# uberalex974/Reinforcement-Learning

Measured on AMD Instinct MI355X. Metric: env-steps/sec (whole node) at 32768 arenas; PPO wall-clock per 1M steps, higher is better.
Workload: dtype f32

## Files before the change

### include/rlgpu_ppo.h

```cpp
#ifndef RLGPU_PPO_H
#define RLGPU_PPO_H

#include <stdint.h>
#include "rlgpu_core.h"

#ifdef __cplusplus
extern "C" {
#endif

#define RLGPU_MAX_LAYERS 8

typedef struct {
    int32_t obs_size;
    int32_t num_actions;
    int32_t policy_layers[RLGPU_MAX_LAYERS];
    int32_t n_policy_layers;
    int32_t critic_layers[RLGPU_MAX_LAYERS];
    int32_t n_critic_layers;
    int32_t layer_norm;
    float leaky_slope;
    int32_t activation;
    float policy_lr, critic_lr;
    float beta1, beta2, eps, weight_decay;
    float clip_range;
// ... 8 lines not shown
    int64_t sample_row_offset;
    float policy_temperature;
    int32_t mask_entropy;
} rlgpu_ppo_config;

enum { RLGPU_GEMM_F32X6 = 0, RLGPU_GEMM_F32 = 1, RLGPU_GEMM_F16X3 = 2 };
enum { RLGPU_ACT_LEAKY_RELU = 0, RLGPU_ACT_RELU = 1, RLGPU_ACT_SIGMOID = 2, RLGPU_ACT_TANH = 3 };
enum { RLGPU_INFER_BF16 = 0, RLGPU_INFER_F16 = 1, RLGPU_INFER_F32 = 2 };

typedef struct rlgpu_ppo rlgpu_ppo;

enum {
    RLGPU_M_ENTROPY = 0, RLGPU_M_KL, RLGPU_M_POLICY_LOSS, RLGPU_M_CRITIC_LOSS, RLGPU_M_RATIO,
    RLGPU_M_CLIP_FRACTION, RLGPU_M_COUNT, RLGPU_M_GRAD_NORM_POLICY, RLGPU_M_GRAD_NORM_CRITIC,
    RLGPU_M_GRAD_NORM_SHARED, RLGPU_M_GUIDING_LOSS = 10 ,
    RLGPU_M_TL_LOSS = 11, RLGPU_M_TL_ACCURACY = 12, RLGPU_M_TL_OLD_ENTROPY = 13,
    RLGPU_M_TL_UPDATE_MAGNITUDE = 14,
    RLGPU_NUM_METRICS = 16
};

int rlgpu_ppo_create(const rlgpu_ppo_config* cfg, rlgpu_ppo** out);
int rlgpu_ppo_destroy(rlgpu_ppo* h);
int32_t rlgpu_ppo_config_size(void);
int rlgpu_ppo_get_config(rlgpu_ppo* h, rlgpu_ppo_config* out);

int rlgpu_ppo_buffers(rlgpu_ppo* h, float** d_params, float** d_grads, int64_t* num_params);
int rlgpu_ppo_model_range(rlgpu_ppo* h, int32_t model, int64_t* offset, int64_t* count);
int rlgpu_ppo_init_params(rlgpu_ppo* h, uint64_t seed, void* stream);
int rlgpu_ppo_refresh_half(rlgpu_ppo* h, void* stream);

int rlgpu_debug_infer_trace(void* d_buf, int64_t capacity);
int rlgpu_kernel_timing(int32_t enable);
int rlgpu_kernel_timing_read(double* ms, double* work, int64_t* count, int32_t nslots);

int rlgpu_ppo_forward(rlgpu_ppo* h, int32_t model, int32_t precision, const float* d_in, int32_t n,
                      float* d_out, void* stream);

int rlgpu_ppo_infer_actions(rlgpu_ppo* h, const float* d_obs, const uint8_t* d_masks, int32_t n,
                            int32_t deterministic, uint64_t rng_step, int32_t* d_actions, float* d_logp,
                            void* stream);
int rlgpu_ppo_set_version(rlgpu_ppo* h, const float* d_policy_params, void* stream);
int rlgpu_ppo_infer_actions_mixed(rlgpu_ppo* h, const float* d_obs, const uint8_t* d_masks, int32_t n,
                                  int32_t deterministic, uint64_t rng_step, const uint8_t* d_old_rows,
                                  int32_t* d_actions, float* d_logp, void* stream);
int rlgpu_ppo_set_guide(rlgpu_ppo* h, const float* d_policy_params, void* stream);
int rlgpu_ppo_infer_guide_logits(rlgpu_ppo* h, const float* d_obs, int64_t n, uint16_t* d_logits16, void* stream);
int rlgpu_ppo_infer_actions_rows(rlgpu_ppo* h, const float* d_obs, const uint8_t* d_masks, int32_t n, int64_t row0,
                                 int32_t deterministic, uint64_t rng_step, const uint8_t* d_old_rows,
                                 int32_t* d_actions, float* d_logp, void* stream);
int rlgpu_ppo_fused_infer(rlgpu_ppo* h, int32_t model);
int rlgpu_ppo_wave_infer(rlgpu_ppo* h, int32_t model);
int rlgpu_ppo_infer_actions_wave(rlgpu_ppo* h, const float* d_obs, const uint8_t* d_masks, int32_t n, int64_t row0,
                                 int32_t deterministic, uint64_t rng_step, const uint8_t* d_old_rows,
                                 int32_t* d_actions, float* d_logp, void* stream);
int rlgpu_ppo_infer_values_wave(rlgpu_ppo* h, int32_t model, const float* d_obs, int32_t n, float* d_out, void* stream);
int rlgpu_ppo_infer_critic(rlgpu_ppo* h, const float* d_obs, int64_t n, float* d_values, void* stream);

int rlgpu_mean_std(const float* d_x, int64_t n, float* d_out, void* stream);

int rlgpu_ppo_minibatch(rlgpu_ppo* h, const float* d_obs, const uint8_t* d_masks, const int32_t* d_actions,
                        const float* d_old_logp, const float* d_adv, const float* d_target,
                        const int32_t* d_index, int64_t start, int32_t n, int64_t batch_size,
                        const float* d_adv_stats, float* d_metrics, void* stream);

int rlgpu_ppo_minibatch_guided(rlgpu_ppo* h, const float* d_obs, const uint8_t* d_masks, const int32_t* d_actions,
                               const float* d_old_logp, const float* d_adv, const float* d_target,
// ... 42 lines not shown
```

### reinforcement-learning_amd/csrc/mlp_kernels.hpp

```cpp
#pragma once
#include <hip/hip_bf16.h>
#include <hip/hip_fp16.h>
#include <hip/hip_runtime.h>
#include <stdint.h>

#include <cstdlib>

namespace mlp {

#define DEV __device__ __forceinline__

typedef float f32x16 __attribute__((ext_vector_type(16)));
typedef short bf16x8 __attribute__((ext_vector_type(8)));

enum { A_IK = 0, A_KI = 1 };
enum { B_JK = 0, B_KJ = 1 };

constexpr int BM = 128, BN = 128, BK = 32;
constexpr int KP = 4;
constexpr int MP = 4;

struct GemmArgs {
    const float* A;
    const float* B;
// ... 1147 lines not shown
                for (int q = 0; q < MAXH; q++) {
                    const int c = lcol<MAXH>(lane, q);
                    v[r][q] = c < H ? z[c] : 0.f;
                }
            }
        }
        lnf_rows<MAXH, RF, ACT>(v, row, R, H, g, b, slope, use_ln, vec, lane, act, stats, vmax, head_w, head_b, head_out);
    }
    if (amax) h3_amax_commit(amax, vmax);
}

constexpr int RLN_BM = 64, RLN_J = 512, RLN_ZP = RLN_J + 8;
constexpr int RLN_LDS = 32 * RLN_ZP * 4;
static_assert(2 * 2 * RLN_BM * 32 * 2 <= RLN_LDS, "the A stages must fit the z stage");
__global__ void __launch_bounds__(256) frag_weight_h3(const uint16_t* planes, int64_t plane, int ld, uint16_t* frag) {
    const int e = blockIdx.x * 256 + threadIdx.x;
    if (e >= (ld / 16) * (RLN_J / 32) * 2 * 64) return;
    const int lane = e & 63, p = (e >> 6) & 1, jb = (e >> 7) % (RLN_J / 32), ks = (e >> 7) / (RLN_J / 32);
    const uint16_t* src = planes + p * plane + (int64_t)(jb * 32 + (lane & 31)) * ld + ks * 16 + 8 * (lane >> 5);
    *reinterpret_cast<u32x4_t*>(frag + (int64_t)e * 8) = *reinterpret_cast<const u32x4_t*>(src);
}
struct RowLnArgs {
    const float* gamma;
    const float* beta;
    float slope;
    int use_ln;
    float* act;
    float2* stats;
    float* amax;
    const float* head_w;
    const float* head_b;
    float* head_out;
};
DEV int h3_row_kloop(const GemmArgs& g, unsigned char* smem, f32x16 (&acc)[2][4]) {
    constexpr int KSTEP = (RLN_J / 32) * 2 * 64 * 8;
    auto As = reinterpret_cast<uint16_t (*)[2][RLN_BM][XK]>(smem);
    const int t = threadIdx.x, lane = t & 63, w = t >> 6;
    const int i0 = blockIdx.x * RLN_BM;
    const int ke = g.K;
#pragma unroll
    for (int a = 0; a < 2; a++)
#pragma unroll
        for (int b = 0; b < 4; b++)
#pragma unroll
            for (int r = 0; r < 16; r++) acc[a][b][r] = 0.f;
    const int srow = t / XKG, kg = t % XKG;
    const float* arow = i0 + srow < g.I ? g.A + (int64_t)(i0 + srow) * g.lda : nullptr;
    f32x4_t va[2];
    const int pa = h3_pow(shard_max_bits(g.amax_a));
    const float sa = pow2f(pa);
    auto load_a = [&](int k0) {
        va[0] = load4v<true>(arow, k0 + kg * 8, ke);
        va[1] = load4v<true>(arow, k0 + kg * 8 + 4, ke);
    };
    auto store_a = [&](int buf) {
        u32x4_t h, l;
        split2h(va, sa, h, l);
        const int c = xchunk<XK>(srow, kg) * 8;
        *reinterpret_cast<u32x4_t*>(&As[buf][0][srow][c]) = h;
        *reinterpret_cast<u32x4_t*>(&As[buf][1][srow][c]) = l;
    };
    const uint16_t* Bw = reinterpret_cast<const uint16_t*>(g.B) + (w * 4 * 2 * 64 + lane) * 8;
    const int last = (int)g.ldb / 16 - 1;
    auto load_b = [&](h16x8 (&b)[2][4], int s) {
        const uint16_t* q = Bw + (int64_t)min(s, last) * KSTEP;
#pragma unroll
        for (int tj = 0; tj < 4; tj++)
#pragma unroll
            for (int p = 0; p < 2; p++) b[p][tj] = *reinterpret_cast<const h16x8*>(q + (tj * 2 + p) * 64 * 8);
    };
    const int l32 = lane & 31, hh = lane >> 5;
    auto mfma_step = [&](int buf, int ks, const h16x8 (&b)[2][4]) {
        const int kc = 2 * ks + hh;
        h16x8 a[2][2];
#pragma unroll
        for (int p = 0; p < 2; p++)
#pragma unroll
            for (int u = 0; u < 2; u++) a[p][u] = kc_frag(As[buf][p], l32 + 32 * u, kc);
        h3_mfma_step<4>(a, b, acc);
    };
    h16x8 b0[2][4], b1[2][4];
    load_a(0);
    load_b(b0, 0);
    store_a(0);
    __syncthreads();
    load_a(XK);
    int buf = 0;
    for (int k0 = 0; k0 < ke; k0 += XK) {
        const int s = k0 / 16;
        load_b(b1, s + 1);
        __builtin_amdgcn_sched_barrier(0);
        mfma_step(buf, 0, b0);
        __builtin_amdgcn_sched_barrier(0);
        load_b(b0, s + 2);
        __builtin_amdgcn_sched_barrier(0);
        mfma_step(buf, 1, b1);
        store_a(buf ^ 1);
        load_a(k0 + 2 * XK);
        __syncthreads();
        buf ^= 1;
    }
    return pa;
}
__global__ void __launch_bounds__(256, 2) gemm_h3_rowln(GemmArgs g, RowLnArgs ln) {
    constexpr int MAXH = RLN_J / 64, RF = lnf_rf<MAXH>();
    __shared__ __attribute__((aligned(16))) unsigned char smem[RLN_LDS];
    float* zs = reinterpret_cast<float*>(smem);
    const int t = threadIdx.x, lane = t & 63, w = t >> 6;
    const int i0 = blockIdx.x * RLN_BM;
    const int l32 = lane & 31, hh = lane >> 5;
    f32x16 acc[2][4];
    const int pa = h3_row_kloop(g, smem, acc);
    float csc[4], bj[4];
#pragma unroll
    for (int tj = 0; tj < 4; tj++) {
        const int j = w * 128 + tj * 32 + l32;
        csc[tj] = g.bscale[j];
        bj[tj] = g.bias ? g.bias[j] : 0.f;
    }
    float lg[MAXH], lb[MAXH];
    lnf_affine<MAXH>(ln.gamma, ln.beta, RLN_J, ln.use_ln, lane, lg, lb);
    uint32_t vmax = 0;
#pragma unroll
    for (int ti = 0; ti < 2; ti++) {
        if (ti) __syncthreads();
#pragma unroll
        for (int tj = 0; tj < 4; tj++)
#pragma unroll
            for (int r = 0; r < 16; r++) {
                const float v = acc[ti][tj][r] + 0.f;
                zs[((r & 3) + 8 * (r >> 2) + 4 * hh) * RLN_ZP + w * 128 + tj * 32 + l32] = h3_out(v, csc[tj], pa, bj[tj]);
            }
        __syncthreads();
        for (int b0 = 0; b0 < 32 / 4; b0 += RF) {
            int row[RF];
            float v[RF][MAXH];
#pragma unroll
            for (int r = 0; r < RF; r++) {
                const int zr = w * (32 / 4) + b0 + r;
                row[r] = i0 + ti * 32 + zr;
#pragma unroll
                for (int q = 0; q < MAXH; q += 4) {
                    const int c = lcol<MAXH>(lane, q);
                    const float4 x = *reinterpret_cast<const float4*>(zs + zr * RLN_ZP + c);
                    v[r][q] = x.x; v[r][q + 1] = x.y; v[r][q + 2] = x.z; v[r][q + 3] = x.w;
                    if (row[r] < g.I) *reinterpret_cast<float4*>(g.C + (int64_t)row[r] * g.ldc + c) = x;
                }
            }
            lnf_rows<MAXH, RF>(v, row, g.I, RLN_J, lg, lb, ln.slope, ln.use_ln, true, lane, ln.act, ln.stats, vmax, ln.head_w,
                               ln.head_b, ln.head_out);
        }
    }
    if (ln.amax) h3_amax_commit(ln.amax, vmax);
}

template <int MAXH>
DEV int hcol(int lane, int q) {
    return MAXH >= 8 ? 8 * lane + 512 * (q >> 3) + (q & 7) : MAXH * lane + q;
}
template <int MAXH, bool F16, int ACT = ACT_LEAKY>
__global__ void __launch_bounds__(256) ln_act_fwd_bf16(const uint16_t* Z, const uint16_t* gamma, const uint16_t* beta, int R,
                                                      int H, float slope, int use_ln, uint16_t* out) {
    const int wv = threadIdx.x >> 6, lane = threadIdx.x & 63;
    const bool vec = (H % 8 == 0) && (MAXH % 8 == 0);
    float g[MAXH], b[MAXH];
#pragma unroll
    for (int q = 0; q < MAXH; q++) {
        const int c = hcol<MAXH>(lane, q);
        g[q] = (use_ln && c < H) ? h2f<F16>(gamma[c]) : 1.f;
        b[q] = (use_ln && c < H) ? h2f<F16>(beta[c]) : 0.f;
    }
    for (int i = 0; i < LNF_ROWS / 4; i++) {
        const int row = blockIdx.x * LNF_ROWS + i * 4 + wv;
        if (row >= R) break;
        const uint16_t* z = Z + (int64_t)row * H;
        float v[MAXH];
        if (vec) {
#pragma unroll
            for (int q = 0; q < MAXH; q += 8) {
                const int c = hcol<MAXH>(lane, q);
                u32x4 t = {0u, 0u, 0u, 0u};
                if (c < H) t = *reinterpret_cast<const u32x4*>(z + c);
#pragma unroll
                for (int k = 0; k < 4; k++) {
                    v[q + 2 * k] = h2f<F16>((uint16_t)(t[k] & 0xffffu));
                    v[q + 2 * k + 1] = h2f<F16>((uint16_t)(t[k] >> 16));
                }
// ... 178 lines not shown
        red[w][2][c] = pb[q];
    }
    __syncthreads();
    if (HEAD) {
#pragma unroll
        for (int q = 0; q < MAXH; q++) hred[w][lcol<MAXH>(lane, q)] = ph[q];
        if (lane == 0) hred[w][64 * MAXH] = phb;
    }
    __syncthreads();
    float* out = part + (int64_t)blockIdx.x * 3 * H;
    for (int k = 0; k < 3; k++)
        for (int c = threadIdx.x; c < H; c += 256)
            out[k * H + c] = red[0][k][c] + red[1][k][c] + red[2][k][c] + red[3][k][c];
    if (HEAD) {
        float* ho = head_part + (int64_t)blockIdx.x * (H + 1);
        for (int c = threadIdx.x; c < H; c += 256) ho[c] = hred[0][c] + hred[1][c] + hred[2][c] + hred[3][c];
        if (threadIdx.x == 0)
            ho[H] = hred[0][64 * MAXH] + hred[1][64 * MAXH] + hred[2][64 * MAXH] + hred[3][64 * MAXH];
    }
    if (amax) h3_amax_commit(amax, vmax);
}

struct RowLnBwdArgs {
    const float* gamma;
    const float* beta;
    float slope;
    int use_ln;
    const float* z;
    const float2* stats;
    float* dz;
    float* part;
    float* amax;
};
__global__ void __launch_bounds__(256, 2) gemm_h3_row_lnbwd(GemmArgs g, RowLnBwdArgs ln) {
    constexpr int MAXH = RLN_J / 64, PR = 2;
    const int H = g.J;
    static_assert(4 * 3 * RLN_J * 4 <= RLN_LDS, "the wave partials must fit the dA stage");
    __shared__ __attribute__((aligned(16))) unsigned char smem[RLN_LDS];
    float* zs = reinterpret_cast<float*>(smem);
    auto red = reinterpret_cast<float (*)[3][RLN_J]>(smem);
    const int t = threadIdx.x, lane = t & 63, w = t >> 6;
    const int i0 = blockIdx.x * RLN_BM;
    const int l32 = lane & 31, hh = lane >> 5;
    f32x16 acc[2][4];
    const int pa = h3_row_kloop(g, smem, acc);
    float csc[4];
#pragma unroll
    for (int tj = 0; tj < 4; tj++) csc[tj] = g.bscale[w * 128 + tj * 32 + l32];
    uint32_t vmax = 0;
#pragma unroll
    for (int ti = 0; ti < 2; ti++) {
        const int r0 = i0 + ti * 32;
        if (ti) {
            if (r0 >= g.I) break;
            __syncthreads();
        }
#pragma unroll
        for (int tj = 0; tj < 4; tj++)
#pragma unroll
            for (int r = 0; r < 16; r++) {
                const float v = acc[ti][tj][r] + 0.f;
                zs[((r & 3) + 8 * (r >> 2) + 4 * hh) * RLN_ZP + w * 128 + tj * 32 + l32] = h3_out(v, csc[tj], pa, 0.f);
            }
        __syncthreads();
        float lg[MAXH], lb[MAXH], pg[MAXH], pb[MAXH], pz[MAXH], ph[MAXH];
        float phb = 0.f;
        lnf_affine<MAXH>(ln.gamma, ln.beta, H, ln.use_ln, lane, lg, lb);
#pragma unroll
        for (int q = 0; q < MAXH; q++) pg[q] = pb[q] = pz[q] = ph[q] = 0.f;
        for (int rr = w; rr < 32; rr += 4 * PR) {
            float xs[PR][MAXH], as[PR][MAXH];
            float2 sts[PR];
#pragma unroll
            for (int j = 0; j < PR; j++) {
                const int row = r0 + rr + 4 * j;
                const int rw = row < g.I ? row : g.I - 1;
                const float* xh = ln.z + (int64_t)rw * H;
                sts[j] = ln.stats[rw];
#pragma unroll
                for (int q = 0; q < MAXH; q += 4) {
                    const int c = lcol<MAXH>(lane, q);
                    const float4 x = *reinterpret_cast<const float4*>(xh + c);
                    const float4 u = *reinterpret_cast<const float4*>(zs + (rr + 4 * j) * RLN_ZP + c);
                    xs[j][q] = x.x; xs[j][q + 1] = x.y; xs[j][q + 2] = x.z; xs[j][q + 3] = x.w;
                    as[j][q] = u.x; as[j][q + 1] = u.y; as[j][q + 2] = u.z; as[j][q + 3] = u.w;
                }
            }
#pragma unroll
            for (int j = 0; j < PR; j++) {
                const int row = r0 + rr + 4 * j;
                if (row >= g.I) break;
                lnb_row<MAXH, false>(xs[j], as[j], sts[j], 0.f, lg, lb, ln.slope, ln.use_ln, H, true, lane,
                                     ln.dz + (int64_t)row * H, pz, pg, pb, ph, phb, vmax);
            }
        }
        __syncthreads();
#pragma unroll
        for (int q = 0; q < MAXH; q += 4) {
            const int c = lcol<MAXH>(lane, q);
            *reinterpret_cast<float4*>(&red[w][0][c]) = make_float4(pz[q], pz[q + 1], pz[q + 2], pz[q + 3]);
            *reinterpret_cast<float4*>(&red[w][1][c]) = make_float4(pg[q], pg[q + 1], pg[q + 2], pg[q + 3]);
            *reinterpret_cast<float4*>(&red[w][2][c]) = make_float4(pb[q], pb[q + 1], pb[q + 2], pb[q + 3]);
        }
        __syncthreads();
        float* out = ln.part + (int64_t)(2 * blockIdx.x + ti) * 3 * H;
#pragma unroll
        for (int k = 0; k < 3; k++)
#pragma unroll
            for (int c = t; c < H; c += 256) out[k * H + c] = red[0][k][c] + red[1][k][c] + red[2][k][c] + red[3][k][c];
    }
    if (ln.amax) h3_amax_commit(ln.amax, vmax);
}

constexpr int LNW_ROWS = 32;
DEV int wcol(int k) { return 4 * (int)threadIdx.x + 1024 * k; }
DEV float4 ld4(const float* p, int c, int H) { return c < H ? *reinterpret_cast<const float4*>(p + c) : make_float4(0.f, 0.f, 0.f, 0.f); }

template <int NV, int ACT = ACT_LEAKY, int LNW_RB = 4>
__global__ void __launch_bounds__(256) ln_act_fwd_wide(const float* Z, const float* gamma, const float* beta, int R, int H,
                                                      float slope, int use_ln, float* act, float2* stats, float* amax,
                                                      const float*, const float*, float*) {
    __shared__ float red[2][LNW_RB][4];
    const int w = threadIdx.x >> 6;
    uint32_t vmax = 0;
    float4 g[NV], b[NV];
#pragma unroll
    for (int k = 0; k < NV; k++) {
        g[k] = use_ln ? ld4(gamma, wcol(k), H) : make_float4(1.f, 1.f, 1.f, 1.f);
        b[k] = use_ln ? ld4(beta, wcol(k), H) : make_float4(0.f, 0.f, 0.f, 0.f);
    }
    const int r_end = min(R, (int)(blockIdx.x + 1) * LNW_ROWS);
    for (int r0 = blockIdx.x * LNW_ROWS; r0 < r_end; r0 += LNW_RB) {
        float4 v[LNW_RB][NV];
#pragma unroll
        for (int j = 0; j < LNW_RB; j++) {
            const float* z = Z + (int64_t)min(r0 + j, R - 1) * H;
#pragma unroll
            for (int k = 0; k < NV; k++) v[j][k] = ld4(z, wcol(k), H);
        }
        float mean[LNW_RB], rs[LNW_RB];
#pragma unroll
        for (int j = 0; j < LNW_RB; j++) {
            mean[j] = 0.f;
            rs[j] = 1.f;
        }
// ... 312 lines not shown
```

### reinforcement-learning_amd/csrc/ppo.hip

```cpp
#include <hipcub/hipcub.hpp>

#include <cmath>
#include <cstring>
#include <type_traits>
#include <vector>

#include "../../include/rlgpu_ppo.h"
#include "common.hpp"
#include "mlp_kernels.hpp"
#include "ppo_kernels.hpp"
#include "infer_kernels.hpp"

namespace {

using rlgpu::ceil_div;

#define RLGPU_H16_LAUNCH(F16, KERN, ...)                                                     \
    do {                                                                                     \
        if (F16) hipLaunchKernelGGL(KERN<true>, __VA_ARGS__);                                \
        else hipLaunchKernelGGL(KERN<false>, __VA_ARGS__);                                   \
    } while (0)

struct Side {
    int64_t planes = -1;
// ... 81 lines not shown
    int nm = 2;
    bool shared() const { return nm == 3; }
    float* dshared = nullptr;
    int64_t nparams = 0, nhalf = 0;
    float *params = nullptr, *grads = nullptr, *exp_avg = nullptr, *exp_avg_sq = nullptr;
    uint16_t* half = nullptr;
    uint16_t* half_ver = nullptr;
    uint16_t *frag = nullptr, *frag_ver = nullptr;
    int64_t nfrag = 0;
    bool has_ver = false;
    uint16_t *half_guide = nullptr, *frag_guide = nullptr;
    float* guide_f = nullptr;
    bool has_guide = false;
    float* teach_f = nullptr;
    bool split_dirty[3] = {true, true, true};
    int64_t step[3] = {0, 0, 0};
    int32_t opt[3] = {RLGPU_OPT_ADAMW, RLGPU_OPT_ADAMW, RLGPU_OPT_ADAMW};
    bool opt_stepped[3] = {false, false, false};
    int hmax = 0;
    float *scratch = nullptr;
    hipStream_t aux = nullptr;
    hipEvent_t ev_fork = nullptr, ev_join = nullptr;
    float* x0 = nullptr;
    int x_ld = 0;
    float* x_amax = nullptr;
    float* amax_all = nullptr;
    int64_t amax_count = 0;
    uint16_t* xh = nullptr;
    int xh_ld = 0;
    uint16_t *zh = nullptr, *ah[2] = {nullptr, nullptr}, *logits_h = nullptr;
    float* logits_f = nullptr;
    std::vector<Link> chain[3];
    bool fused_fit[3] = {false, false, false};
    std::vector<void*> allocs;

    template <class T>
    T* alloc(size_t count) {
        allocs.push_back(nullptr);
        allocs.back() = rlgpu::dev_alloc(count * sizeof(T) + 16);
        return (T*)allocs.back();
    }
};

inline bool f16(const rlgpu_ppo* h) { return h->cfg.infer_fp16 == RLGPU_INFER_F16; }
inline bool infer_f32(const rlgpu_ppo* h) { return h->cfg.infer_fp16 == RLGPU_INFER_F32; }

namespace {

namespace ktime {
enum { FWD_GEMM = 0, WGRAD_GEMM = 1, LN_FWD = 2, LN_BWD = 3, NSLOT = 4 };
struct Rec {
    hipEvent_t a, b;
    int slot;
    double work;
};
struct State {
    bool on = false;
    std::vector<Rec> recs;
    std::vector<hipEvent_t> pool;
};
State g;
hipEvent_t event() {
    hipEvent_t e;
    if (!g.pool.empty()) {
        e = g.pool.back();
        g.pool.pop_back();
// ... 240 lines not shown
    if (S.planes >= 0)
        gemm_x6_pre(a, m.wsplit + S.planes, S.ld, S.plane(), wscale_at(m, S.scale), C, J, bias, n, J, K, s);
    else
        gemm_f32(m.mode, mlp::A_IK, bwd ? mlp::B_KJ : mlp::B_JK, a, Operand{P + L.w, L.in, nullptr, false}, C, J, bias, n, J, K, 1, s);
}

mlp::GemmArgs row_args(const Model& m, const Side& S, const Operand& a, int n, int K) {
    return gemm_args(true, a, m.wsplit + S.frag, S.ld, nullptr, wscale_at(m, S.scale), n, mlp::RLN_J, K, mlp::RLN_BM, mlp::RLN_J);
}

void forward_train(rlgpu_ppo* h, int mi, const Operand& x, int n, float* out, hipStream_t s) {
    Model& m = h->M[mi];
    const float* P = h->params;
    if (h->split_dirty[mi]) {
        split_weights(P, m, s);
        h->split_dirty[mi] = false;
    }
    const int nh = nhid(m);
    const Layer* O = m.head_only ? nullptr : &m.L[nh];
    const bool head1 = O && O->out == 1;
    Operand in = x;
    for (int l = 0; l < nh; l++) {
        const Layer& L = m.L[l];
        const bool fuse = head1 && l == nh - 1;
        const mlp::RowLnArgs ln{L.g >= 0 ? P + L.g : nullptr, L.be >= 0 ? P + L.be : nullptr, h->cfg.leaky_slope, h->cfg.layer_norm,
                                m.act[l], reinterpret_cast<float2*>(m.rstd[l]), amax_slot(m, l), fuse ? P + O->w : nullptr,
                                fuse ? P + O->b : nullptr, fuse ? out : nullptr};
        if (rowfuse_fwd(m, L) && vec_ok(in, L.in)) {
            ktime::Span span(ktime::FWD_GEMM, 2.0 * n * L.out * L.in, s);
            mlp::GemmArgs g = row_args(m, L.fwd, in, n, L.in);
            g.C = m.xhat[l];
            g.bias = P + L.b;
            g.ldc = L.out;
            launch_gemm(mlp::gemm_h3_rowln, 256, s, g, ln);
        } else {
            linear(P, m, L, false, in, n, m.xhat[l], s);
            ktime::Span span(ktime::LN_FWD, (double)n * (8.0 * L.out + 8.0), s);
            int lnf_rows = 0;
            const auto lnf = mlp::ln_act_fwd_f32_pick(m.akind, L.out, &lnf_rows, fuse);
            hipLaunchKernelGGL(lnf, dim3(ceil_div(n, lnf_rows)), dim3(256), 0, s, m.xhat[l], ln.gamma, ln.beta, n, L.out, ln.slope,
                               ln.use_ln, ln.act, ln.stats, ln.amax, ln.head_w, ln.head_b, ln.head_out);
            RLGPU_CHECK_HIP(hipGetLastError());
        }
        in = Operand{m.act[l], L.out, amax_slot(m, l), false};
    }
    if (O && !head1) linear(P, m, *O, false, in, n, out, s);
}

bool dA_ln_bwd_fused(rlgpu_ppo* h, Model& m, int l, const Operand& a, int n, float* dz_out, hipStream_t s) {
    if (l < 1) return false;
    const Layer& L = m.L[l];
    const Layer& C = m.L[l - 1];
    if (!rowfuse_bwd(m, L, &C) || !vec_ok(a, L.out)) return false;
    const float* P = h->params;
    ktime::Span span(ktime::FWD_GEMM, 2.0 * n * L.in * L.out, s);
    const mlp::GemmArgs g = row_args(m, L.bwd, a, n, L.out);
    const mlp::RowLnBwdArgs ln{C.g >= 0 ? P + C.g : nullptr, C.be >= 0 ? P + C.be : nullptr, h->cfg.leaky_slope, h->cfg.layer_norm,
                               m.xhat[l - 1], reinterpret_cast<const float2*>(m.rstd[l - 1]), dz_out, m.cpart_l[l - 1],
                               amax_slot(m, kAmaxDZ + l - 1)};
    launch_gemm(mlp::gemm_h3_row_lnbwd, 256, s, g, ln);
    return true;
}

void backward(rlgpu_ppo* h, int mi, const Operand& x, int n, const float* dout, hipStream_t s,
              const float* dout_part = nullptr, int dout_nblk = 0) {
    Model& m = h->M[mi];
    const float* P = h->params;
    float* G = h->grads;
    const int nh = nhid(m);
    const auto input_of = [&](int l) { return l > 0 ? Operand{m.act[l - 1], m.L[l].in, amax_slot(m, l - 1), false} : x; };
    const float* dA_top = m.dA;
    bool rank1 = false;
    float* fused_dz = nullptr;
    Reducer R;
    R.m = &m;
    const Layer* O = m.head_only ? nullptr : &m.L[nh];
    if (!O) {
        dA_top = dout;
    } else if (O->out == 1) {
        rank1 = true;
    } else {
        if (!dout_part) throw rlgpu::Error(RLGPU_ERR_STATE, "backward: a multi-column dout needs the loss kernel's bias partials");
        const int dld = dout_ld(O->out);
        const Operand d{dout, dld, amax_slot(m, kAmaxOut), dld > O->out};
        weight_grad(m, d, O->out, input_of(nh), O->in, n, G + O->w, s, R, m.wpart_l[nh]);
        R.add(dout_part, dout_nblk, O->out, O->out, G + O->b, false, s);
        if (dA_ln_bwd_fused(h, m, nh, d, n, m.dZ, s)) fused_dz = m.dZ;
        else linear(P, m, *O, true, d, n, m.dA, s);
    }
    const float* dA_in = dA_top;
    for (int l = nh - 1; l >= 0; l--) {
        const Layer& L = m.L[l];
        const float* gg = L.g >= 0 ? P + L.g : nullptr;
// ... 559 lines not shown
    });
}

extern "C" int rlgpu_ppo_infer_actions(rlgpu_ppo* h, const float* d_obs, const uint8_t* d_masks, int32_t n,
                                       int32_t deterministic, uint64_t rng_step, int32_t* d_actions, float* d_logp,
                                       void* stream) {
    return rlgpu::guarded([&] {
        RLGPU_REQUIRE(h && d_obs && d_masks && d_actions, "null argument");
        RLGPU_REQUIRE(n >= 0, "n must be >= 0");
        infer_policy(h, Rows{d_obs, n, h->cfg.sample_row_offset, d_masks}, Draw{deterministic, rng_step, d_actions, d_logp},
                     nullptr, h->cfg.max_rows, rlgpu::as_stream(stream));
    });
}

extern "C" int rlgpu_debug_infer_trace(void* d_buf, int64_t capacity) {
    return rlgpu::guarded([&] {
        RLGPU_REQUIRE(!d_buf || capacity >= 16, "rlgpu_debug_infer_trace: capacity below one workgroup's 16 marks");
        g_infer_trace = (unsigned long long*)d_buf;
        g_infer_trace_cap = d_buf ? capacity : 0;
    });
}

extern "C" int rlgpu_ppo_set_version(rlgpu_ppo* h, const float* d_policy_params, void* stream) {
    return rlgpu::guarded([&] {
        RLGPU_REQUIRE(h && d_policy_params, "rlgpu_ppo_set_version: null argument");
        hipStream_t s = rlgpu::as_stream(stream);
        half_from(h, 0, d_policy_params, h->half_ver, h->frag_ver, s);
        if (h->shared()) half_from(h, 2, d_policy_params + h->M[0].count, h->half_ver, h->frag_ver, s);
        h->has_ver = true;
    });
}

static_assert(ppo::kGuidingLossSlot == RLGPU_M_GUIDING_LOSS, "the guided loss kernel's metric slot");

extern "C" int rlgpu_ppo_set_guide(rlgpu_ppo* h, const float* d_policy_params, void* stream) {
    return rlgpu::guarded([&] {
        RLGPU_REQUIRE(h && d_policy_params, "rlgpu_ppo_set_guide: null argument");
        if (infer_f32(h))
            throw rlgpu::Error(RLGPU_ERR_UNSUPPORTED, "rlgpu_ppo_set_guide: fp32 inference (RLGPU_INFER_F32) keeps no 16-bit "
                                                      "copies (a guiding policy needs 16-bit inference)");
        hipStream_t s = rlgpu::as_stream(stream);
        if (!h->half_guide) {
            h->half_guide = h->alloc<uint16_t>(h->nhalf + 8);
            h->frag_guide = h->alloc<uint16_t>(h->nfrag);
            h->guide_f = h->alloc<float>((int64_t)h->cfg.max_rows * h->cfg.num_actions);
        }
        half_from(h, 0, d_policy_params, h->half_guide, h->frag_guide, s);
        if (h->shared()) half_from(h, 2, d_policy_params + h->M[0].count, h->half_guide, h->frag_guide, s);
        h->has_guide = true;
    });
}

extern "C" int rlgpu_ppo_infer_guide_logits(rlgpu_ppo* h, const float* d_obs, int64_t n, uint16_t* d_logits16, void* stream) {
    return rlgpu::guarded([&] {
        RLGPU_REQUIRE(h && d_obs && d_logits16 && n >= 0, "rlgpu_ppo_infer_guide_logits: bad argument");
        RLGPU_REQUIRE(h->has_guide, "rlgpu_ppo_infer_guide_logits: no guide set (rlgpu_ppo_set_guide)");
        hipStream_t s = rlgpu::as_stream(stream);
        const int A = h->cfg.num_actions;
        const Rows rows{d_obs, n, 0, nullptr};
        for (int64_t b = 0; b < n; b += h->cfg.max_rows) {
            const Rows r = rows.sub(h->cfg, b, std::min<int64_t>(h->cfg.max_rows, n - b));
            const int64_t e = r.n * A;
            uint16_t* out = d_logits16 + b * A;
            if (fused_ok(h, 0)) {
                infer_fused(h, 0, Weights::Guide, r, h->guide_f, nullptr, s);
                RLGPU_H16_LAUNCH(f16(h), ppo::to_half, dim3(ceil_div(e, 256)), dim3(256), 0, s, h->guide_f, out, e);
// ... 522 lines not shown
```

### reinforcement-learning_amd/rlgpu/ppo.py

```python
import ctypes
import math

from . import _lib
from ._lib import alias

MAX_LAYERS = 8
NUM_METRICS = 16
METRICS = ("entropy", "kl", "policy_loss", "critic_loss", "ratio", "clip_fraction", "count",
           "grad_norm_policy", "grad_norm_critic", "grad_norm_shared", "guiding_loss", "tl_loss", "tl_accuracy",
           "tl_old_entropy")
M_GUIDING_LOSS = 10
M_TL_LOSS, M_TL_ACCURACY, M_TL_OLD_ENTROPY = 11, 12, 13
MODEL_NAMES = ("policy", "critic", "shared_head")


class _Cfg(ctypes.Structure):
    _fields_ = [("obs_size", ctypes.c_int32), ("num_actions", ctypes.c_int32),
                ("policy_layers", ctypes.c_int32 * MAX_LAYERS), ("n_policy_layers", ctypes.c_int32),
                ("critic_layers", ctypes.c_int32 * MAX_LAYERS), ("n_critic_layers", ctypes.c_int32),
                ("layer_norm", ctypes.c_int32), ("leaky_slope", ctypes.c_float), ("activation", ctypes.c_int32),
                ("policy_lr", ctypes.c_float), ("critic_lr", ctypes.c_float),
                ("beta1", ctypes.c_float), ("beta2", ctypes.c_float), ("eps", ctypes.c_float),
                ("weight_decay", ctypes.c_float), ("clip_range", ctypes.c_float),
                ("entropy_scale", ctypes.c_float), ("max_grad_norm", ctypes.c_float),
# ... 36 lines not shown
    L.rlgpu_ppo_config_size.restype = i32
    L.rlgpu_ppo_buffers.argtypes = [vp, ctypes.POINTER(vp), ctypes.POINTER(vp), ctypes.POINTER(i64)]
    L.rlgpu_ppo_model_range.argtypes = [vp, i32, ctypes.POINTER(i64), ctypes.POINTER(i64)]
    L.rlgpu_ppo_init_params.argtypes = [vp, u64, vp]
    L.rlgpu_ppo_refresh_half.argtypes = [vp, vp]
    L.rlgpu_ppo_forward.argtypes = [vp, i32, i32, vp, i32, vp, vp]
    L.rlgpu_ppo_infer_actions.argtypes = [vp, vp, vp, i32, i32, u64, vp, vp, vp]
    L.rlgpu_ppo_infer_critic.argtypes = [vp, vp, i64, vp, vp]
    L.rlgpu_mean_std.argtypes = [vp, i64, vp, vp]
    L.rlgpu_ppo_minibatch.argtypes = [vp, vp, vp, vp, vp, vp, vp, vp, i64, i32, i64, vp, vp, vp]
    L.rlgpu_ppo_minibatch_guided.argtypes = [vp, vp, vp, vp, vp, vp, vp, vp, i64, i32, i64, vp, vp, f32, vp, vp]
    L.rlgpu_ppo_set_guide.argtypes = [vp, vp, vp]
    L.rlgpu_ppo_infer_guide_logits.argtypes = [vp, vp, i64, vp, vp]
    L.rlgpu_ppo_optimizer_step.argtypes = [vp, vp, vp]
    L.rlgpu_ppo_zero_grad.argtypes = [vp, vp]
    L.rlgpu_ppo_optimizer_state.argtypes = [vp, ctypes.POINTER(i64), ctypes.POINTER(vp), ctypes.POINTER(vp)]
    L.rlgpu_ppo_set_optimizer_step.argtypes = [vp, i64]
    L.rlgpu_ppo_model_optimizer_step.argtypes = [vp, i32, ctypes.POINTER(i64)]
    L.rlgpu_ppo_set_model_optimizer_step.argtypes = [vp, i32, i64]
    L.rlgpu_ppo_set_optimizer.argtypes = [vp, i32, i32]
    L.rlgpu_ppo_get_optimizer.argtypes = [vp, i32, ctypes.POINTER(i32)]
    L.rlgpu_ppo_teacher_probs.argtypes = [vp, vp, vp, i64, vp, i32, vp, vp, vp, vp]
    L.rlgpu_teacher_probs_from_logits.argtypes = [vp, vp, i64, i32, vp, i32, f32, i32, vp, vp, vp, vp]
    L.rlgpu_ppo_transfer_chunk.argtypes = [vp, vp, vp, vp, vp, vp, i64, i32, i64, i32, f32, f32, vp, vp]
    L.rlgpu_ppo_transfer_step.argtypes = [vp, f32, vp]
    L.rlgpu_diff_norm.argtypes = [vp, vp, i64, vp, vp, vp]
    L.rlgpu_ppo_set_version.argtypes = [vp, vp, vp]
    L.rlgpu_ppo_infer_actions_mixed.argtypes = [vp, vp, vp, i32, i32, u64, vp, vp, vp, vp]
    L.rlgpu_ppo_infer_actions_rows.argtypes = [vp, vp, vp, i32, i64, i32, u64, vp, vp, vp, vp]
    L.rlgpu_ppo_infer_actions_wave.argtypes = [vp, vp, vp, i32, i64, i32, u64, vp, vp, vp, vp]
    L.rlgpu_ppo_infer_values_wave.argtypes = [vp, i32, vp, i32, vp, vp]
    L.rlgpu_ppo_wave_infer.argtypes = [vp, i32]
    L.rlgpu_permutation.argtypes = [i64, u64, u64, vp, vp]
    L.rlgpu_kernel_timing.argtypes = [i32]
    L.rlgpu_kernel_timing_read.argtypes = [vp, vp, vp, i32]
    _bound = True
    return L


def param_count(obs_size, num_actions, layers, out=None, layer_norm=True):
    n, prev = 0, obs_size
    for h in layers:
        n += prev * h + h + (2 * h if layer_norm else 0)
        prev = h
    o = num_actions if out is None else out
    return n + prev * o + o


class PPO:

    def __init__(self, obs_size=167, num_actions=90, policy_layers=(512, 512), critic_layers=(512, 512),
                 layer_norm=True, policy_lr=2.5e-4, critic_lr=2.5e-4, clip_range=0.2, entropy_scale=0.035,
                 max_grad_norm=0.5, max_rows=50_000, seed=42, init=True, device="cuda:0",
                 betas=(0.9, 0.999), eps=1e-8, weight_decay=1e-2, leaky_slope=0.01, train_gemm=GEMM_F16X3,
                 infer_fp16=False, shared_layers=(), policy_temperature=1.0, mask_entropy=False, activation="leaky_relu",
                 optimizer="adamw"):
        import torch
        opt_type = optimizer_id(optimizer)
        if optimizer == "adam":
            weight_decay = 0.0
        if not torch.cuda.is_available():
            raise _lib.RLGPUError("PPO needs an MI355X: the product path has no CPU fallback")
        L = _bind()
        self.device = torch.device(device)
        torch.cuda.set_device(self.device)
        c = _Cfg()
# ... 159 lines not shown
    def forward(self, model, x, half=False, out=None):
        import torch
        n = x.shape[0]
        width = self.model_out(model)
        out = torch.empty((n, width), device=self.device) if out is None else out
        _lib.check(_lib.lib().rlgpu_ppo_forward(self._h, model, int(half), _lib.ptr(x.contiguous()), n, _lib.ptr(out),
                                                _lib.stream_ptr()), "rlgpu_ppo_forward")
        return out

    def infer_actions(self, obs, masks, step=0, deterministic=False, actions=None, logp=None):
        import torch
        n = obs.shape[0]
        actions = torch.empty(n, dtype=torch.int32, device=self.device) if actions is None else actions
        logp = torch.empty(n, device=self.device) if logp is None else logp
        _lib.check(_lib.lib().rlgpu_ppo_infer_actions(self._h, _lib.ptr(obs), _lib.ptr(masks), n, int(deterministic),
                                                      step, _lib.ptr(actions), _lib.ptr(logp), _lib.stream_ptr()),
                   "rlgpu_ppo_infer_actions")
        return actions, logp

    def set_version(self, policy_params):
        cnt = sum(self.model_range(m)[1] for m in self.models if m != 1)
        if policy_params.numel() != cnt:
            raise _lib.RLGPUError("policy version has the wrong parameter count")
        _lib.check(_lib.lib().rlgpu_ppo_set_version(self._h, _lib.ptr(policy_params.contiguous()), _lib.stream_ptr()),
                   "rlgpu_ppo_set_version")

    def set_guide(self, policy_params):
        cnt = sum(self.model_range(m)[1] for m in self.models if m != 1)
        if policy_params.numel() != cnt:
            raise _lib.RLGPUError("guiding policy has the wrong parameter count")
        _lib.check(_lib.lib().rlgpu_ppo_set_guide(self._h, _lib.ptr(policy_params.contiguous()), _lib.stream_ptr()),
                   "rlgpu_ppo_set_guide")

    @property
    def logit_dtype(self):
        import torch
        return torch.float16 if self.infer_fp16 == 1 else torch.bfloat16

    def guide_logits(self, obs, out=None):
        import torch
        n = obs.shape[0]
        out = torch.empty((n, self.num_actions), dtype=self.logit_dtype, device=self.device) if out is None else out
        _lib.check(_lib.lib().rlgpu_ppo_infer_guide_logits(self._h, _lib.ptr(obs.contiguous()), n, _lib.ptr(out),
                                                           _lib.stream_ptr()), "rlgpu_ppo_infer_guide_logits")
        return out

    def infer_actions_mixed(self, obs, masks, old_rows, step=0, deterministic=False, actions=None, logp=None):
        import torch
        n = obs.shape[0]
        actions = torch.empty(n, dtype=torch.int32, device=self.device) if actions is None else actions
        logp = torch.empty(n, device=self.device) if logp is None else logp
        _lib.check(_lib.lib().rlgpu_ppo_infer_actions_mixed(self._h, _lib.ptr(obs), _lib.ptr(masks), n, int(deterministic),
                                                            step, _lib.ptr(old_rows), _lib.ptr(actions), _lib.ptr(logp),
                                                            _lib.stream_ptr()), "rlgpu_ppo_infer_actions_mixed")
        return actions, logp

    def _actions_rows(self, entry, obs, masks, row0, step, deterministic, old_rows, actions, logp):
        import torch
        n = obs.shape[0]
        actions = torch.empty(n, dtype=torch.int32, device=self.device) if actions is None else actions
        logp = torch.empty(n, device=self.device) if logp is None else logp
        _lib.check(getattr(_lib.lib(), entry)(self._h, _lib.ptr(obs), _lib.ptr(masks), n, row0, int(deterministic), step,
                                              _lib.ptr(old_rows) if old_rows is not None else None, _lib.ptr(actions),
                                              _lib.ptr(logp), _lib.stream_ptr()), entry)
        return actions, logp

# ... 153 lines not shown
                first = self.metrics.clone()
            self.transfer_step(cfg.lr)
        self.metrics.zero_()
        rep = {"Old Policy Entropy": float(tm[M_TL_OLD_ENTROPY])}
        if first is not None:
            rep.update({"Transfer Learn Accuracy": float(first[M_TL_ACCURACY]), "Transfer Learn Loss": float(first[M_TL_LOSS]),
                        "Policy Entropy": float(first[0])})
        rep["Policy Update Magnitude"] = diff_norm(before, self.model_slice(0))
        return rep

    def model_sizes(self, model):
        return [p.numel() for p in self.torch_module(model).parameters()]


def make_sequential(obs_size, out, layers, layer_norm=True, leaky_slope=0.01, activation="leaky_relu"):
    import torch
    act = (lambda: torch.nn.LeakyReLU(leaky_slope), torch.nn.ReLU, torch.nn.Sigmoid, torch.nn.Tanh)[activation_id(activation)]
    mods, prev = [], obs_size
    for hdim in layers:
        mods.append(torch.nn.Linear(prev, hdim))
        if layer_norm:
            mods.append(torch.nn.LayerNorm(hdim))
        mods.append(act())
        prev = hdim
    if out is not None:
        mods.append(torch.nn.Linear(prev, out))
    return torch.nn.Sequential(*mods)


KERNEL_TIMING_SLOTS = ("forward / input-gradient GEMMs", "weight-gradient GEMMs", "LayerNorm forward",
                       "LayerNorm backward")


def kernel_timing(enable):
    _bind()
    _lib.check(_lib.lib().rlgpu_kernel_timing(1 if enable else 0), "rlgpu_kernel_timing")


def kernel_timing_read():
    import numpy as np
    _bind()
    n = len(KERNEL_TIMING_SLOTS)
    ms, work, cnt = np.zeros(n), np.zeros(n), np.zeros(n, np.int64)
    _lib.check(_lib.lib().rlgpu_kernel_timing_read(ms.ctypes.data, work.ctypes.data, cnt.ctypes.data, n),
               "rlgpu_kernel_timing_read")
    return {k: (float(ms[i]), float(work[i]), int(cnt[i])) for i, k in enumerate(KERNEL_TIMING_SLOTS)}


def teacher_probs_from_logits(logits, masks, temperature=1.0, mask_entropy=False, action_map=None, metrics=None):
    import torch
    _bind()
    n, a_old = logits.shape
    A = a_old if action_map is None else action_map.shape[-1]
    probs = torch.empty((n, A), device=logits.device)
    arg = torch.empty(n, dtype=torch.int32, device=logits.device)
    _lib.check(_lib.lib().rlgpu_teacher_probs_from_logits(
        _lib.ptr(logits.contiguous()), _lib.ptr(masks.contiguous()), n, a_old,
        _lib.ptr(action_map.contiguous()) if action_map is not None else None, A, temperature, int(mask_entropy),
        _lib.ptr(probs), _lib.ptr(arg), _lib.ptr(metrics) if metrics is not None else None, _lib.stream_ptr()),
        "rlgpu_teacher_probs_from_logits")
    return probs, arg


def diff_norm(a, b):
    import torch
    _bind()
# ... 17 lines not shown
```

Before: 2.439 million.

## Prefetch LN constants and backward rows during K-loop; add per-phase row-kernel profiler

```diff
diff --git a/include/rlgpu_ppo.h b/include/rlgpu_ppo.h
--- a/include/rlgpu_ppo.h
+++ b/include/rlgpu_ppo.h
@@ -64,6 +64,8 @@
 int rlgpu_debug_infer_trace(void* d_buf, int64_t capacity);
 int rlgpu_kernel_timing(int32_t enable);
 int rlgpu_kernel_timing_read(double* ms, double* work, int64_t* count, int32_t nslots);
+#define RLGPU_ROW_SPLIT_SLOTS 16
+int rlgpu_ppo_set_row_split(rlgpu_ppo* h, unsigned long long* d_slots, int64_t capacity);
 
 int rlgpu_ppo_forward(rlgpu_ppo* h, int32_t model, int32_t precision, const float* d_in, int32_t n,
                       float* d_out, void* stream);
diff --git a/reinforcement-learning_amd/csrc/mlp_kernels.hpp b/reinforcement-learning_amd/csrc/mlp_kernels.hpp
--- a/reinforcement-learning_amd/csrc/mlp_kernels.hpp
+++ b/reinforcement-learning_amd/csrc/mlp_kernels.hpp
@@ -1203,7 +1203,62 @@
     const float* head_b;
     float* head_out;
 };
-DEV int h3_row_kloop(const GemmArgs& g, unsigned char* smem, f32x16 (&acc)[2][4]) {
+enum {
+    kRowCount = 0,
+    kRowK = 1,
+    kRowRows = 2,
+    kRowKind = 3,
+    kRowTotal = 4,
+    kRowPrologue = 5,
+    kRowKLoop = 6,
+    kRowBarrier = 7,
+    kRowStage0 = 8,
+    kRowPasses0 = 9,
+    kRowPart0 = 10,
+    kRowExit = 14,
+    kRowSlots = 16
+};
+template <bool ON>
+struct RowClock;
+template <>
+struct RowClock<false> {
+    DEV void mark(int) {}
+    DEV void wait_begin() {}
+    DEV void wait_end() {}
+    DEV void finish(int, int, int) {}
+};
+template <>
+struct RowClock<true> {
+    unsigned long long* slot;
+    unsigned long long t_in, last, w0, waited;
+    DEV explicit RowClock(unsigned long long* s) : slot(s + (size_t)blockIdx.x * kRowSlots), waited(0) { t_in = last = wall_clock64(); }
+    DEV void mark(int k) {
+        const unsigned long long now = wall_clock64();
+        if (threadIdx.x == 0) atomicAdd(slot + k, now - last);
+        last = wall_clock64();
+    }
+    DEV void wait_begin() { w0 = wall_clock64(); }
+    DEV void wait_end() { waited += wall_clock64() - w0; }
+    DEV void finish(int kind, int K, int rows) {
+        const unsigned long long now = wall_clock64();
+        if (threadIdx.x == 0) {
+            atomicAdd(slot + kRowTotal, now - t_in);
+            atomicAdd(slot + kRowBarrier, waited);
+            atomicAdd(slot + kRowCount, 1ull);
+            slot[kRowK] = (unsigned long long)K;
+            slot[kRowRows] = (unsigned long long)rows;
+            slot[kRowKind] = (unsigned long long)kind;
+        }
+    }
+};
+
+struct RowConst {
+    const float* p;
+    float dflt;
+};
+template <bool SPLIT, int NC>
+DEV int h3_row_kloop(const GemmArgs& g, unsigned char* smem, f32x16 (&acc)[2][4], RowClock<SPLIT>& clk, const RowConst (&cs)[NC],
+                     float (*park)[RLN_J]) {
     constexpr int KSTEP = (RLN_J / 32) * 2 * 64 * 8;
     auto As = reinterpret_cast<uint16_t (*)[2][RLN_BM][XK]>(smem);
     const int t = threadIdx.x, lane = t & 63, w = t >> 6;
@@ -1253,8 +1308,19 @@
     h16x8 b0[2][4], b1[2][4];
     load_a(0);
     load_b(b0, 0);
+    float cv[NC][RLN_J / 256];
+#pragma unroll
+    for (int n = 0; n < NC; n++)
+#pragma unroll
+        for (int u = 0; u < RLN_J / 256; u++)
+            cv[n][u] = *(cs[n].p ? cs[n].p + t + 256 * u : reinterpret_cast<const float*>(g_zero_row));
     store_a(0);
+#pragma unroll
+    for (int n = 0; n < NC; n++)
+#pragma unroll
+        for (int u = 0; u < RLN_J / 256; u++) park[n][t + 256 * u] = cs[n].p ? cv[n][u] : cs[n].dflt;
     __syncthreads();
+    clk.mark(kRowPrologue);
     load_a(XK);
     int buf = 0;
     for (int k0 = 0; k0 < ke; k0 += XK) {
@@ -1268,12 +1334,17 @@
         mfma_step(buf, 1, b1);
         store_a(buf ^ 1);
         load_a(k0 + 2 * XK);
+        clk.wait_begin();
         __syncthreads();
+        clk.wait_end();
         buf ^= 1;
     }
+    clk.mark(kRowKLoop);
     return pa;
 }
-__global__ void __launch_bounds__(256, 2) gemm_h3_rowln(GemmArgs g, RowLnArgs ln) {
+template <bool SPLIT, class... Slots>
+__global__ void __launch_bounds__(256, 2) gemm_h3_rowln(GemmArgs g, RowLnArgs ln, Slots... slots) {
+    RowClock<SPLIT> clk(slots...);
     constexpr int MAXH = RLN_J / 64, RF = lnf_rf<MAXH>();
     __shared__ __attribute__((aligned(16))) unsigned char smem[RLN_LDS];
     float* zs = reinterpret_cast<float*>(smem);
@@ -1281,16 +1352,22 @@
     const int i0 = blockIdx.x * RLN_BM;
     const int l32 = lane & 31, hh = lane >> 5;
     f32x16 acc[2][4];
-    const int pa = h3_row_kloop(g, smem, acc);
+    __shared__ __attribute__((aligned(16))) float cpark[4][RLN_J];
+    const RowConst consts[4] = {{g.bscale, 0.f}, {g.bias, 0.f}, {ln.use_ln ? ln.gamma : nullptr, 1.f}, {ln.use_ln ? ln.beta : nullptr, 0.f}};
+    const int pa = h3_row_kloop(g, smem, acc, clk, consts, cpark);
     float csc[4], bj[4];
 #pragma unroll
     for (int tj = 0; tj < 4; tj++) {
         const int j = w * 128 + tj * 32 + l32;
-        csc[tj] = g.bscale[j];
-        bj[tj] = g.bias ? g.bias[j] : 0.f;
+        csc[tj] = cpark[0][j];
+        bj[tj] = cpark[1][j];
     }
     float lg[MAXH], lb[MAXH];
-    lnf_affine<MAXH>(ln.gamma, ln.beta, RLN_J, ln.use_ln, lane, lg, lb);
+#pragma unroll
+    for (int q = 0; q < MAXH; q++) {
+        lg[q] = cpark[2][lcol<MAXH>(lane, q)];
+        lb[q] = cpark[3][lcol<MAXH>(lane, q)];
+    }
     uint32_t vmax = 0;
 #pragma unroll
     for (int ti = 0; ti < 2; ti++) {
@@ -1303,6 +1380,7 @@
                 zs[((r & 3) + 8 * (r >> 2) + 4 * hh) * RLN_ZP + w * 128 + tj * 32 + l32] = h3_out(v, csc[tj], pa, bj[tj]);
             }
         __syncthreads();
+        clk.mark(kRowStage0 + 3 * ti);
         for (int b0 = 0; b0 < 32 / 4; b0 += RF) {
             int row[RF];
             float v[RF][MAXH];
@@ -1321,9 +1399,13 @@
             lnf_rows<MAXH, RF>(v, row, g.I, RLN_J, lg, lb, ln.slope, ln.use_ln, true, lane, ln.act, ln.stats, vmax, ln.head_w,
                                ln.head_b, ln.head_out);
         }
+        clk.mark(kRowPasses0 + 3 * ti);
     }
     if (ln.amax) h3_amax_commit(ln.amax, vmax);
-}
+    clk.mark(kRowExit);
+    clk.finish(0, g.K, min(RLN_BM, g.I - i0));
+}
+template __global__ void gemm_h3_rowln<false>(GemmArgs, RowLnArgs);
 
 template <int MAXH>
 DEV int hcol(int lane, int q) {
@@ -1568,7 +1650,9 @@
     float* part;
     float* amax;
 };
-__global__ void __launch_bounds__(256, 2) gemm_h3_row_lnbwd(GemmArgs g, RowLnBwdArgs ln) {
+template <bool SPLIT, class... Slots>
+__global__ void __launch_bounds__(256, 2) gemm_h3_row_lnbwd(GemmArgs g, RowLnBwdArgs ln, Slots... slots) {
+    RowClock<SPLIT> clk(slots...);
     constexpr int MAXH = RLN_J / 64, PR = 2;
     const int H = g.J;
     static_assert(4 * 3 * RLN_J * 4 <= RLN_LDS, "the wave partials must fit the dA stage");
@@ -1579,10 +1663,40 @@
     const int i0 = blockIdx.x * RLN_BM;
     const int l32 = lane & 31, hh = lane >> 5;
     f32x16 acc[2][4];
-    const int pa = h3_row_kloop(g, smem, acc);
+    __shared__ __attribute__((aligned(16))) float cpark[3][RLN_J];
+    const RowConst consts[3] = {{g.bscale, 0.f}, {ln.use_ln ? ln.gamma : nullptr, 1.f}, {ln.use_ln ? ln.beta : nullptr, 0.f}};
+    const int pa = h3_row_kloop(g, smem, acc, clk, consts, cpark);
+    const float* __restrict__ zsrc = ln.z;
+    const float2* __restrict__ stsrc = ln.stats;
+    float* __restrict__ dzdst = ln.dz;
+    float* __restrict__ pdst = ln.part;
+    struct Pass {
+        float4 x[PR][MAXH / 4];
+        float2 st[PR];
+    };
+    auto request = [&](int ti, int p, Pass& q) {
+#pragma unroll
+        for (int j = 0; j < PR; j++) {
+            const int row = i0 + ti * 32 + w + 8 * p + 4 * j;
+            const int rw = row < g.I ? row : g.I - 1;
+            const float* xh = zsrc + (int64_t)rw * H;
+            q.st[j] = stsrc[rw];
+#pragma unroll
+            for (int k = 0; k < MAXH / 4; k++) q.x[j][k] = *reinterpret_cast<const float4*>(xh + lcol<MAXH>(lane, 4 * k));
+        }
+    };
+    Pass nxt;
+    request(0, 0, nxt);
     float csc[4];
 #pragma unroll
-    for (int tj = 0; tj < 4; tj++) csc[tj] = g.bscale[w * 128 + tj * 32 + l32];
+    for (int tj = 0; tj < 4; tj++) csc[tj] = cpark[0][w * 128 + tj * 32 + l32];
+    float lg[MAXH], lb[MAXH];
+#pragma unroll
+    for (int q = 0; q < MAXH; q++) {
+        const int c = lcol<MAXH>(lane, q);
+        lg[q] = c < H ? cpark[1][c] : 1.f;
+        lb[q] = c < H ? cpark[2][c] : 0.f;
+    }
     uint32_t vmax = 0;
 #pragma unroll
     for (int ti = 0; ti < 2; ti++) {
@@ -1599,24 +1713,24 @@
                 zs[((r & 3) + 8 * (r >> 2) + 4 * hh) * RLN_ZP + w * 128 + tj * 32 + l32] = h3_out(v, csc[tj], pa, 0.f);
             }
         __syncthreads();
-        float lg[MAXH], lb[MAXH], pg[MAXH], pb[MAXH], pz[MAXH], ph[MAXH];
+        clk.mark(kRowStage0 + 3 * ti);
+        float pg[MAXH], pb[MAXH], pz[MAXH], ph[MAXH];
         float phb = 0.f;
-        lnf_affine<MAXH>(ln.gamma, ln.beta, H, ln.use_ln, lane, lg, lb);
 #pragma unroll
         for (int q = 0; q < MAXH; q++) pg[q] = pb[q] = pz[q] = ph[q] = 0.f;
-        for (int rr = w; rr < 32; rr += 4 * PR) {
+#pragma unroll
+        for (int p = 0; p < 32 / (4 * PR); p++) {
+            const int rr = w + 4 * PR * p;
+            const Pass cur = nxt;
+            if (p + 1 < 32 / (4 * PR)) request(ti, p + 1, nxt);
+            else if (ti == 0) request(1, 0, nxt);
             float xs[PR][MAXH], as[PR][MAXH];
-            float2 sts[PR];
 #pragma unroll
             for (int j = 0; j < PR; j++) {
-                const int row = r0 + rr + 4 * j;
-                const int rw = row < g.I ? row : g.I - 1;
-                const float* xh = ln.z + (int64_t)rw * H;
-                sts[j] = ln.stats[rw];
 #pragma unroll
                 for (int q = 0; q < MAXH; q += 4) {
                     const int c = lcol<MAXH>(lane, q);
-                    const float4 x = *reinterpret_cast<const float4*>(xh + c);
+                    const float4 x = cur.x[j][q / 4];
                     const float4 u = *reinterpret_cast<const float4*>(zs + (rr + 4 * j) * RLN_ZP + c);
                     xs[j][q] = x.x; xs[j][q + 1] = x.y; xs[j][q + 2] = x.z; xs[j][q + 3] = x.w;
                     as[j][q] = u.x; as[j][q + 1] = u.y; as[j][q + 2] = u.z; as[j][q + 3] = u.w;
@@ -1626,10 +1740,11 @@
             for (int j = 0; j < PR; j++) {
                 const int row = r0 + rr + 4 * j;
                 if (row >= g.I) break;
-                lnb_row<MAXH, false>(xs[j], as[j], sts[j], 0.f, lg, lb, ln.slope, ln.use_ln, H, true, lane,
-                                     ln.dz + (int64_t)row * H, pz, pg, pb, ph, phb, vmax);
-            }
-        }
+                lnb_row<MAXH, false>(xs[j], as[j], cur.st[j], 0.f, lg, lb, ln.slope, ln.use_ln, H, true, lane,
+                                     dzdst + (int64_t)row * H, pz, pg, pb, ph, phb, vmax);
+            }
+        }
+        clk.mark(kRowPasses0 + 3 * ti);
         __syncthreads();
 #pragma unroll
         for (int q = 0; q < MAXH; q += 4) {
@@ -1639,14 +1754,18 @@
             *reinterpret_cast<float4*>(&red[w][2][c]) = make_float4(pb[q], pb[q + 1], pb[q + 2], pb[q + 3]);
         }
         __syncthreads();
-        float* out = ln.part + (int64_t)(2 * blockIdx.x + ti) * 3 * H;
+        float* out = pdst + (int64_t)(2 * blockIdx.x + ti) * 3 * H;
 #pragma unroll
         for (int k = 0; k < 3; k++)
 #pragma unroll
             for (int c = t; c < H; c += 256) out[k * H + c] = red[0][k][c] + red[1][k][c] + red[2][k][c] + red[3][k][c];
+        clk.mark(kRowPart0 + 3 * ti);
     }
     if (ln.amax) h3_amax_commit(ln.amax, vmax);
-}
+    clk.mark(kRowExit);
+    clk.finish(1, g.K, min(RLN_BM, g.I - i0));
+}
+template __global__ void gemm_h3_row_lnbwd<false>(GemmArgs, RowLnBwdArgs);
 
 constexpr int LNW_ROWS = 32;
 DEV int wcol(int k) { return 4 * (int)threadIdx.x + 1024 * k; }
diff --git a/reinforcement-learning_amd/csrc/ppo.hip b/reinforcement-learning_amd/csrc/ppo.hip
--- a/reinforcement-learning_amd/csrc/ppo.hip
+++ b/reinforcement-learning_amd/csrc/ppo.hip
@@ -137,6 +137,13 @@
     float* logits_f = nullptr;
     std::vector<Link> chain[3];
     bool fused_fit[3] = {false, false, false};
+    unsigned long long* d_row_split = nullptr;
+    int64_t row_split_recs = 0, row_split_n = 0;
+    int64_t row_split_wg() const { return rlgpu::ceil_div(cfg.max_rows, mlp::RLN_BM); }
+    unsigned long long* row_split_next() {
+        if (!d_row_split) return nullptr;
+        return d_row_split + (row_split_n++ % row_split_recs) * row_split_wg() * mlp::kRowSlots;
+    }
     std::vector<void*> allocs;
 
     template <class T>
@@ -443,7 +450,8 @@
             g.C = m.xhat[l];
             g.bias = P + L.b;
             g.ldc = L.out;
-            launch_gemm(mlp::gemm_h3_rowln, 256, s, g, ln);
+            if (unsigned long long* rec = h->row_split_next()) launch_gemm(mlp::gemm_h3_rowln<true, unsigned long long*>, 256, s, g, ln, rec);
+            else launch_gemm(mlp::gemm_h3_rowln<false>, 256, s, g, ln);
         } else {
             linear(P, m, L, false, in, n, m.xhat[l], s);
             ktime::Span span(ktime::LN_FWD, (double)n * (8.0 * L.out + 8.0), s);
@@ -469,7 +477,8 @@
     const mlp::RowLnBwdArgs ln{C.g >= 0 ? P + C.g : nullptr, C.be >= 0 ? P + C.be : nullptr, h->cfg.leaky_slope, h->cfg.layer_norm,
                                m.xhat[l - 1], reinterpret_cast<const float2*>(m.rstd[l - 1]), dz_out, m.cpart_l[l - 1],
                                amax_slot(m, kAmaxDZ + l - 1)};
-    launch_gemm(mlp::gemm_h3_row_lnbwd, 256, s, g, ln);
+    if (unsigned long long* rec = h->row_split_next()) launch_gemm(mlp::gemm_h3_row_lnbwd<true, unsigned long long*>, 256, s, g, ln, rec);
+    else launch_gemm(mlp::gemm_h3_row_lnbwd<false>, 256, s, g, ln);
     return true;
 }
 
@@ -1095,6 +1104,19 @@
 }
 
 static_assert(ppo::kGuidingLossSlot == RLGPU_M_GUIDING_LOSS, "the guided loss kernel's metric slot");
+static_assert(mlp::kRowSlots == RLGPU_ROW_SPLIT_SLOTS, "the full-row kernels' profiled slots");
+
+extern "C" int rlgpu_ppo_set_row_split(rlgpu_ppo* h, unsigned long long* d_slots, int64_t capacity) {
+    return rlgpu::guarded([&] {
+        RLGPU_REQUIRE(h, "rlgpu_ppo_set_row_split: null handle");
+        const int64_t rec = (int64_t)mlp::kRowSlots * h->row_split_wg();
+        RLGPU_REQUIRE(!d_slots || capacity >= rec, "rlgpu_ppo_set_row_split: buffer of " + std::to_string(capacity) +
+                                                       " slots, one launch record needs " + std::to_string(rec));
+        h->d_row_split = d_slots;
+        h->row_split_recs = d_slots ? capacity / rec : 0;
+        h->row_split_n = 0;
+    });
+}
 
 extern "C" int rlgpu_ppo_set_guide(rlgpu_ppo* h, const float* d_policy_params, void* stream) {
     return rlgpu::guarded([&] {
diff --git a/reinforcement-learning_amd/rlgpu/ppo.py b/reinforcement-learning_amd/rlgpu/ppo.py
--- a/reinforcement-learning_amd/rlgpu/ppo.py
+++ b/reinforcement-learning_amd/rlgpu/ppo.py
@@ -92,6 +92,7 @@
     L.rlgpu_ppo_infer_values_wave.argtypes = [vp, i32, vp, i32, vp, vp]
     L.rlgpu_ppo_wave_infer.argtypes = [vp, i32]
     L.rlgpu_permutation.argtypes = [i64, u64, u64, vp, vp]
+    L.rlgpu_ppo_set_row_split.argtypes = [vp, vp, i64]
     L.rlgpu_kernel_timing.argtypes = [i32]
     L.rlgpu_kernel_timing_read.argtypes = [vp, vp, vp, i32]
     _bound = True
@@ -317,6 +318,10 @@
         _lib.check(_lib.lib().rlgpu_ppo_set_guide(self._h, _lib.ptr(policy_params.contiguous()), _lib.stream_ptr()),
                    "rlgpu_ppo_set_guide")
 
+    def set_row_split(self, slots):
+        _lib.check(_lib.lib().rlgpu_ppo_set_row_split(self._h, _lib.ptr(slots), 0 if slots is None else slots.numel()),
+                   "rlgpu_ppo_set_row_split")
+
     @property
     def logit_dtype(self):
         import torch
@@ -536,6 +541,11 @@
                        "LayerNorm backward")
 
 
+ROW_SPLIT_SLOTS = 16
+ROW_SPLIT_NAMES = ("count", "K", "rows", "kind", "total", "prologue", "kloop", "kloop_barrier", "stage0", "passes0", "part0",
+                   "stage1", "passes1", "part1", "exit", "unused")
+
+
 def kernel_timing(enable):
     _bind()
     _lib.check(_lib.lib().rlgpu_kernel_timing(1 if enable else 0), "rlgpu_kernel_timing")
```

After: 2.458 million, median of 6. No clear change (+0.8%).
